# shanjiayao/PTT

Measured on AMD Instinct MI355X. Metric: tracklet frames/sec (hot path: PointNet++ SA stack + Point-Track-Transformer blocks), higher is better.
Workload: dtype f32

## Files before the change

### include/ptt_hip.h

```cpp
#ifndef PTT_HIP_H
#define PTT_HIP_H

#include <stddef.h>
#include <stdint.h>

#ifdef __cplusplus
extern "C" {
#endif

#define PTT_ABI_VERSION 28

enum {
    PTT_OK = 0,
    PTT_EINVAL = -1,
    PTT_EUNSUPPORTED = -2,
    PTT_ELAUNCH = -3,
    PTT_EWORKSPACE = -4
};

typedef void* ptt_stream_t;

int ptt_version(void);
const char* ptt_error_name(int code);
const char* ptt_last_error_string(void);

// ... 3 lines not shown
                   size_t workspace_elems, ptt_stream_t stream);

int ptt_gather_f32(const float* feat, const int32_t* idx, int B, int C, int N, int M,
                   float* out, ptt_stream_t stream);
int ptt_gather_grad_f32(const float* grad_out, const int32_t* idx, int B, int C, int N,
                        int M, float* grad_feat, ptt_stream_t stream);

int ptt_select_centres_f32(const float* xyz, const int32_t* idx, int B, int N, int M, float* new_xyz,
                           int64_t* idx64_out, ptt_stream_t stream);

int ptt_ball_query_f32(const float* new_xyz, const float* xyz, int B, int M, int N,
                       float radius, int nsample, int32_t* idx_out, ptt_stream_t stream);

int ptt_centres_ball_query_f32(const float* xyz, const int32_t* sel, int B, int N, int M, float radius, int nsample,
                               float* new_xyz, int64_t* idx64_out, int32_t* idx_out, ptt_stream_t stream);

int ptt_group_f32(const float* feat, const int32_t* idx, int B, int C, int N, int M,
                  int ns, float* out, ptt_stream_t stream);
int ptt_group_grad_f32(const float* grad_out, const int32_t* idx, int B, int C, int N,
                       int M, int ns, float* grad_feat, ptt_stream_t stream);

size_t ptt_scatter_add_det_workspace(int B, int N, int E);
int ptt_scatter_add_det_f32(const float* src, const int32_t* idx, int B, int C, int N, int E, float* out,
                            void* workspace, size_t workspace_bytes, ptt_stream_t stream);

int ptt_knn_f32(const float* xyz, int B, int N, int k, int32_t* idx_out,
                ptt_stream_t stream);
int ptt_knn_rel_f32(const float* xyz, int B, int N, int k, int32_t* idx_out, float* rel_out,
                    ptt_stream_t stream);

// ... 66 lines not shown
    int64_t feat_sb, feat_sc, feat_sn;
    float* out;
    int64_t out_sb, out_sc, out_sm;
    int B, N, M, nsample, C;
    float radius;
    int use_xyz;
    int normalize_xyz;
    int n_layers;
    ptt_sa_layer layers[PTT_SA_MAX_LAYERS];
    const float* l0_point_term;
    const float* l0_xyz_weight;
    int l0_channels;
    int l0_relu;
    void* compact_ws;
    size_t compact_ws_bytes;
} ptt_sa_desc;

int ptt_sa_fused_fwd_f32(const ptt_sa_desc* d, ptt_stream_t stream);
size_t ptt_sa_compact_workspace(int B, int M);

typedef struct ptt_xcorr_desc {
    const float* cos_t;
    const float* P;
    const float* w_sim;
    const float* scale0;
    const float* shift0;
    float* out;
    int64_t out_sb, out_sc, out_sn;
    float* sim_out;
    int B, Ns, Nt, C0;
    int n_layers;
    ptt_sa_layer layers[PTT_SA_MAX_LAYERS];
    int32_t split; int64_t out_sh;
    const float* search_feat; const float* templ_feat;
// ... 361 lines not shown
```

### ptt_amd/_lib.py

```python
import ctypes
import os
import re
from ctypes import Structure, c_char_p, c_double, c_float, c_int, c_int32, c_int64, c_longlong, c_size_t, c_uint32, c_void_p

from .build import HEADER as HEADER_PATH, LIB as LIB_PATH


def _strip_comments(text):
    return re.sub(r"/\*.*?\*/|//[^\n]*", " ", text, flags=re.S)


def parse_defines(text):
    return {n: int(v) for n, v in re.findall(r"^[ \t]*#[ \t]*define[ \t]+(PTT_\w+)[ \t]+(-?\d+)[ \t]*$", _strip_comments(text), re.M)}


CTYPES = {"int": c_int, "int32_t": c_int32, "uint32_t": c_uint32, "int64_t": c_int64, "long long": c_longlong, "size_t": c_size_t,
          "float": c_float, "double": c_double, "ptt_stream_t": c_void_p}


def _ctype(decl, name, is_return=False):
    words = decl.replace("*", " * ").split()
    if not is_return and len(words) > 1 and words[-1] != "*":
        words.pop()
    if "*" in words:
# ... 135 lines not shown


class SaLayer(Structure):
    _fields_ = [("Wpacked", c_void_p), ("scale", c_void_p), ("shift", c_void_p),
                ("Cin", c_int), ("Cout", c_int), ("relu", c_int)]


class SaDesc(Structure):
    _fields_ = [("xyz", c_void_p), ("new_xyz", c_void_p), ("idx", c_void_p), ("feat", c_void_p),
                ("feat_sb", c_int64), ("feat_sc", c_int64), ("feat_sn", c_int64),
                ("out", c_void_p), ("out_sb", c_int64), ("out_sc", c_int64), ("out_sm", c_int64),
                ("B", c_int), ("N", c_int), ("M", c_int), ("nsample", c_int), ("C", c_int),
                ("radius", c_float), ("use_xyz", c_int), ("normalize_xyz", c_int), ("n_layers", c_int),
                ("layers", SaLayer * PTT_SA_MAX_LAYERS),
                ("l0_point_term", c_void_p), ("l0_xyz_weight", c_void_p), ("l0_channels", c_int), ("l0_relu", c_int),
                ("compact_ws", c_void_p), ("compact_ws_bytes", c_size_t)]


class XcorrDesc(Structure):
    _fields_ = [("cos_t", c_void_p), ("P", c_void_p), ("w_sim", c_void_p), ("scale0", c_void_p), ("shift0", c_void_p),
                ("out", c_void_p), ("out_sb", c_int64), ("out_sc", c_int64), ("out_sn", c_int64),
                ("sim_out", c_void_p),
                ("B", c_int), ("Ns", c_int), ("Nt", c_int), ("C0", c_int),
                ("n_layers", c_int), ("layers", SaLayer * PTT_SA_MAX_LAYERS),
                ("split", c_int32), ("out_sh", c_int64), ("search_feat", c_void_p), ("templ_feat", c_void_p),
                ("s_sb", c_int64), ("s_sn", c_int64), ("t_sb", c_int64), ("t_sn", c_int64), ("C", c_int), ("eps", c_float)]


class AttnDesc(Structure):
    _fields_ = [("xyz", c_void_p), ("rel", c_void_p), ("knn", c_void_p), ("qkv", c_void_p),
                ("Wd1p", c_void_p), ("Wd2p", c_void_p), ("bd2", c_void_p),
# ... 36 lines not shown
```

### ptt_amd/csrc/mfma_ops.hip

```cpp
#include <math.h>
#include <stdlib.h>
#include <string.h>
#include "common.h"
#include "mfma_common.h"

#ifndef PTT_PAIR_PF
#define PTT_PAIR_PF 1
#endif
#ifndef PTT_GATHER_BATCH
#define PTT_GATHER_BATCH 16
#endif
#ifndef PTT_SA_WAVES
#define PTT_SA_WAVES 2
#endif

namespace ptt {

#ifdef PTT_DEV
#define PTT_STAMP(i) do { if (p.dbg && threadIdx.x == 0 && blockIdx.x < 4096) p.dbg[blockIdx.x * 8 + (i)] = __builtin_readcyclecounter(); } while (0)
#else
#define PTT_STAMP(i) do { } while (0)
#endif

__device__ __forceinline__ void stagger_second_slot(int first_wave_blocks, int quanta) {
// ... 1315 lines not shown
            if (valid) tab.ndist()[g0 + lc] = nd;
        }
    }
    __syncthreads();
    if (t < 4) s_base[t] = s_cnt[t] ? atomicAdd(&tab.ws[t], s_cnt[t]) : 0;
    __syncthreads();
    for (int e = t; e < 32 * 32; e += 256) {
        const int lc = e >> 5, j = e & 31, k = s_cls[lc];
        if (k < 0 || j >= (4 << k)) continue;
        const int q = s_base[k] + s_pos[lc];
        tab.rows(k)[(size_t)q * (4 << k) + j] = s_row[lc][j < s_nd[lc] ? j : 0];
        if (j == 0) tab.list(k)[q] = g0 + lc;
    }
}

#ifndef PTT_SAL_WGS
#define PTT_SAL_WGS 1
#endif
#ifndef PTT_SAL_WAVES
#define PTT_SAL_WAVES 12
#endif

template <int ROWS>
struct SacTileT {
    static constexpr int LG = ROWS == 32 ? 3 : 4;
    static_assert(ROWS == 32 || ROWS == 64, "32- or 64-row tiles");
    int k, first, n;
    __device__ __forceinline__ static void count(const int32_t* ws, int total, int (&cnt)[4], int (&tiles)[4]) {
#pragma unroll
        for (int k = 0; k < 4; ++k) {
// ... 665 lines not shown
        cin = s.Cout;
    }
    if (ldo < cin || (residual && ldr < cin)) return fail(PTT_EINVAL, "ptt_rows_mlp_f32: ldo=%d ldr=%d Cout=%d", ldo, ldr, cin);
    p.ldk = maxk + 4;
    p.vec_in = ((K & 3) == 0 && (ldx & 3) == 0 && (reinterpret_cast<uintptr_t>(X) & 15) == 0) ? 1 : 0;
    const int lds = 32 * p.ldk * (int)sizeof(float);
    int rc = set_lds_limit(reinterpret_cast<const void*>(rows_mlp_kernel), lds);
    if (rc) return rc;
    hipLaunchKernelGGL(rows_mlp_kernel, dim3((rows + 31) / 32), dim3(256), lds, as_stream(stream), p);
    return check_launch("rows_mlp_kernel");
}

extern "C" size_t ptt_sa_compact_workspace(int B, int M) {
    const long long T = (long long)(B > 0 ? B : 0) * (M > 0 ? M : 0);
    return SacTable::words((size_t)T) * sizeof(int32_t);
}

extern "C" int ptt_sa_fused_fwd_f32(const ptt_sa_desc* d, ptt_stream_t stream) {
    if (!d) return fail(PTT_EINVAL, "ptt_sa_fused_fwd_f32: null descriptor");
    if (d->B < 0 || d->N <= 0 || d->M < 0 || d->C < 0 || d->n_layers < 1 || d->n_layers > PTT_SA_MAX_LAYERS)
        return fail(PTT_EINVAL, "ptt_sa_fused_fwd_f32: B=%d N=%d M=%d C=%d layers=%d", d->B, d->N, d->M, d->C,
                    d->n_layers);
    if (d->nsample != 16 && d->nsample != 32 && d->nsample != 64)
        return fail(PTT_EUNSUPPORTED, "ptt_sa_fused_fwd_f32: nsample=%d (16, 32 and 64 are instantiated)", d->nsample);
    if (d->B == 0 || d->M == 0) return PTT_OK;
    const bool hoist = d->l0_point_term != nullptr;
    if (!d->xyz || !d->new_xyz || !d->idx || !d->out || (!hoist && d->C > 0 && !d->feat))
        return fail(PTT_EINVAL, "ptt_sa_fused_fwd_f32: null pointer");
    if (!d->use_xyz && d->C == 0) return fail(PTT_EINVAL, "ptt_sa_fused_fwd_f32: no xyz and no features");
    if (hoist) {
// ... 100 lines not shown
        }
        return check_launch("sa_wave_kernel");
    }
    if (p.hoist == 2 && d->nsample == 32 && d->n_layers == 2 && p.L[0].Cin == 128 && p.L[0].Cout == 128 &&
        p.L[1].Cout == 256 && !p.L[0].scale && !p.L[1].scale && p.L[0].relu && dev_switches().sa_stream) {
        p.tiles = (total_centres + 1) / 2;
        int wgs = p.tiles < 512 ? p.tiles : 512;
        p.chunk = (p.tiles + wgs - 1) / wgs;
        if (dev_switches().sa_chunk > 0 && p.chunk > dev_switches().sa_chunk) p.chunk = dev_switches().sa_chunk;
        wgs = (p.tiles + p.chunk - 1) / p.chunk;
        if (d->compact_ws) {
            if (d->compact_ws_bytes < ptt_sa_compact_workspace(d->B, d->M) || (reinterpret_cast<uintptr_t>(d->compact_ws) & 15))
                return fail(PTT_EWORKSPACE, "ptt_sa_fused_fwd_f32: compact_ws needs %zu bytes, 16-byte aligned (got %zu)",
                            ptt_sa_compact_workspace(d->B, d->M), d->compact_ws_bytes);
            p.cws = static_cast<int32_t*>(d->compact_ws);
            hipLaunchKernelGGL(sa_compact_zero_kernel, dim3(1), dim3(64), 0, s, p.cws);
            if ((rc = check_launch("sa_compact_zero_kernel"))) return rc;
            hipLaunchKernelGGL(sa_compact_kernel<false>, dim3((total_centres + 31) / 32), dim3(256), 0, s, d->xyz, d->idx, d->N, d->M,
                               SacTable{p.cws, total_centres});
            if ((rc = check_launch("sa_compact_kernel"))) return rc;
            const int lds = (2 * SAS_TILE + 64 * 4 + 64) * (int)sizeof(float);
            if ((rc = set_lds_limit(reinterpret_cast<const void*>(sa_stream_compact_kernel), lds))) return rc;
            hipLaunchKernelGGL(sa_stream_compact_kernel, dim3(p.tiles < 512 ? p.tiles : 512), dim3(256), lds, s, p);
            return check_launch("sa_stream_compact_kernel");
        }
        const int lds = (2 * SAS_TILE + 4 * 16 * 4) * (int)sizeof(float);
        if ((rc = set_lds_limit(reinterpret_cast<const void*>(sa_stream_kernel<32>), lds))) return rc;
        hipLaunchKernelGGL((sa_stream_kernel<32>), dim3(wgs), dim3(256), lds, s, p);
        return check_launch("sa_stream_kernel");
    }
    int RT = dev_switches().sa_rt;
    if (d->nsample == 64) RT = 2;
    const int lds = 32 * RT * p.ldk * (int)sizeof(float);
    if (lds > 160 * 1024) return fail(PTT_EUNSUPPORTED, "ptt_sa_fused_fwd_f32: %d B of LDS per workgroup", lds);
    const int cpw = 32 * RT / d->nsample;
// ... 126 lines not shown
```

### ptt_amd/csrc/point_ops.hip

```cpp
#pragma clang fp contract(off)

#include <limits.h>
#include <stdlib.h>
#include "common.h"

namespace ptt {

__device__ __forceinline__ float sqdist3(float ax, float ay, float az, float bx, float by, float bz) {
    const float dx = ax - bx, dy = ay - by, dz = az - bz;
    return (dx * dx + dy * dy) + dz * dz;
}

__device__ __forceinline__ float knn_dist(float ax, float ay, float az, float bx, float by, float bz) {
    const float d = sqdist3(ax, ay, az, bx, by, bz);
    return d < __builtin_inff() ? d : 3.402823466e+38f;
}

__device__ __forceinline__ float lane_bcast(float v, int src_lane) {
    return __builtin_bit_cast(float, __builtin_amdgcn_readlane(__builtin_bit_cast(int, v), src_lane));
}

typedef float fps_f2 __attribute__((ext_vector_type(2)));


// ... 181 lines not shown
            PTT_FPS_ABL_CASE(1) PTT_FPS_ABL_CASE(2) PTT_FPS_ABL_CASE(3) PTT_FPS_ABL_CASE(4) PTT_FPS_ABL_CASE(8) PTT_FPS_ABL_CASE(12) PTT_FPS_ABL_CASE(15)
            PTT_FPS_ABL_CASE(16) PTT_FPS_ABL_CASE(32) PTT_FPS_ABL_CASE(47) PTT_FPS_ABL_CASE(7) PTT_FPS_ABL_CASE(24) PTT_FPS_ABL_CASE(40)
#undef PTT_FPS_ABL_CASE
        }
#endif
        hipLaunchKernelGGL((fps_kernel<T, P, true>), dim3(B), dim3(T), sel_bytes + (size_t)N * 12, s, xyz, N, npoint, idx);
        return check_launch("fps_kernel");
    }
    hipLaunchKernelGGL((fps_kernel<T, P, false>), dim3(B), dim3(T), sel_bytes, s, xyz, N, npoint, idx);
    return check_launch("fps_kernel");
}

template <int CPW>
__device__ __forceinline__ void ball_sweep(const float* __restrict__ pts, int N, float r2, int ns, const float (&cx)[CPW],
                                           const float (&cy)[CPW], const float (&cz)[CPW], int ncentres,
                                           int32_t* __restrict__ out0, int lane) {
    int cnt[CPW], first[CPW];
#pragma unroll
    for (int c = 0; c < CPW; ++c) { cnt[c] = (c < ncentres) ? 0 : ns; first[c] = 0; }
    for (int base = 0; base < N; base += 64) {
        const int k = base + lane;
        const bool in = k < N;
        float px = 0.f, py = 0.f, pz = 0.f;
        if (in) { px = pts[3 * k + 0]; py = pts[3 * k + 1]; pz = pts[3 * k + 2]; }
        bool active = false;
#pragma unroll
        for (int c = 0; c < CPW; ++c) {
            if (cnt[c] >= ns) continue;
            const float d = sqdist3(cx[c], cy[c], cz[c], px, py, pz);
            const bool hit = in && d < r2;
            const unsigned long long mask = __ballot(hit);
            if (mask != 0ull) {
                if (cnt[c] == 0) first[c] = base + (__ffsll((long long)mask) - 1);
                const int pos = cnt[c] + __popcll(mask & ((1ull << lane) - 1ull));
                if (hit && pos < ns) out0[(size_t)c * ns + pos] = k;
                cnt[c] += __popcll(mask);
            }
            active = active || cnt[c] < ns;
        }
        if (!active) break;
    }
#pragma unroll
    for (int c = 0; c < CPW; ++c) {
        if (c >= ncentres) break;
        const int fill = (cnt[c] > 0) ? first[c] : 0;
        for (int s = cnt[c] + lane; s < ns; s += 64) out0[(size_t)c * ns + s] = fill;
    }
}

template <int CPW>
__global__ __launch_bounds__(256) void ball_query_kernel(const float* __restrict__ new_xyz,
                                                         const float* __restrict__ xyz, int BM, int M, int N,
                                                         float r2, int ns, int32_t* __restrict__ idx_out) {
    const int centre = (blockIdx.x * 4 + (threadIdx.x >> 6)) * CPW;
    if (centre >= BM) return;
    const int lane = threadIdx.x & 63;
    const int b = centre / M;
    float cx[CPW], cy[CPW], cz[CPW];
    const int nc = min(CPW, BM - centre);
#pragma unroll
    for (int c = 0; c < CPW; ++c) {
        const int cc = centre + (c < nc ? c : 0);
        cx[c] = new_xyz[(size_t)cc * 3 + 0]; cy[c] = new_xyz[(size_t)cc * 3 + 1]; cz[c] = new_xyz[(size_t)cc * 3 + 2];
    }
    ball_sweep<CPW>(xyz + (size_t)b * N * 3, N, r2, ns, cx, cy, cz, nc, idx_out + (size_t)centre * ns, lane);
}

template <int CPW>
__global__ __launch_bounds__(256) void centres_ball_query_kernel(const float* __restrict__ xyz, const int32_t* __restrict__ sel,
                                                                 int BM, int M, int N, float r2, int ns,
                                                                 float* __restrict__ new_xyz, long long* __restrict__ idx64,
                                                                 int32_t* __restrict__ idx_out) {
    const int centre = (blockIdx.x * 4 + (threadIdx.x >> 6)) * CPW;
    if (centre >= BM) return;
    const int lane = threadIdx.x & 63;
    const int b = centre / M;
    const float* __restrict__ pts = xyz + (size_t)b * N * 3;
    float cx[CPW], cy[CPW], cz[CPW];
    const int nc = min(CPW, BM - centre);
#pragma unroll
    for (int c = 0; c < CPW; ++c) {
        const int cc = centre + (c < nc ? c : 0);
        const int n = sel ? sel[cc] : cc - b * M;
        cx[c] = pts[3 * n + 0]; cy[c] = pts[3 * n + 1]; cz[c] = pts[3 * n + 2];
        if (lane == 0 && c < nc) {
            new_xyz[(size_t)cc * 3 + 0] = cx[c]; new_xyz[(size_t)cc * 3 + 1] = cy[c]; new_xyz[(size_t)cc * 3 + 2] = cz[c];
            if (idx64) idx64[cc] = n;
        }
    }
    ball_sweep<CPW>(pts, N, r2, ns, cx, cy, cz, nc, idx_out + (size_t)centre * ns, lane);
}

__global__ void gather_kernel(const float* __restrict__ feat, const int32_t* __restrict__ idx, int C, int N, int M,
                              float* __restrict__ out, size_t total) {
    for (size_t e = (size_t)blockIdx.x * blockDim.x + threadIdx.x; e < total; e += (size_t)gridDim.x * blockDim.x) {
        const int j = (int)(e % M);
        const size_t bc = e / M;
        const int b = (int)(bc / C);
        out[e] = feat[bc * N + idx[(size_t)b * M + j]];
    }
}
__global__ void gather_grad_kernel(const float* __restrict__ go, const int32_t* __restrict__ idx, int C, int N, int M,
                                   float* __restrict__ gf, size_t total) {
    for (size_t e = (size_t)blockIdx.x * blockDim.x + threadIdx.x; e < total; e += (size_t)gridDim.x * blockDim.x) {
        const int j = (int)(e % M);
// ... 852 lines not shown
    if (!xyz || !new_xyz || !idx_out) return fail(PTT_EINVAL, "ptt_centres_ball_query_f32: null pointer");
    const int BM = B * M;
    const int cpw = ball_cpw(BM, M);
    if (cpw == 8)
        hipLaunchKernelGGL((centres_ball_query_kernel<8>), dim3((BM / 8 + 3) / 4), dim3(256), 0, as_stream(stream), xyz, sel, BM,
                           M, N, radius * radius, nsample, new_xyz, reinterpret_cast<long long*>(idx64_out), idx_out);
    else if (cpw == 4)
        hipLaunchKernelGGL((centres_ball_query_kernel<4>), dim3((BM / 4 + 3) / 4), dim3(256), 0, as_stream(stream), xyz, sel, BM,
                           M, N, radius * radius, nsample, new_xyz, reinterpret_cast<long long*>(idx64_out), idx_out);
    else
        hipLaunchKernelGGL((centres_ball_query_kernel<1>), dim3((BM + 3) / 4), dim3(256), 0, as_stream(stream), xyz, sel, BM, M,
                           N, radius * radius, nsample, new_xyz, reinterpret_cast<long long*>(idx64_out), idx_out);
    return check_launch("centres_ball_query_kernel");
}


extern "C" size_t ptt_ball_query_grid_workspace(int B, int N) {
    if (B <= 0 || N <= 0) return 0;
    return (size_t)B * grid_slice_ints(N) * sizeof(int32_t);
}

static int ball_query_grid_launch(const char* who, const float* xyz, const float* centres, const int32_t* sel, int sel_mode, int B, int N, int M,
                                  float radius, int nsample, float* new_xyz, int64_t* idx64, int32_t* idx_out, void* ws, size_t ws_bytes,
                                  ptt_stream_t stream) {
    if (B < 0 || M < 0 || N <= 0 || nsample <= 0) return fail(PTT_EINVAL, "%s: B=%d M=%d N=%d nsample=%d", who, B, M, N, nsample);
    if (B == 0 || M == 0) return PTT_OK;
    if (N > 131072) return fail(PTT_EUNSUPPORTED, "%s: N=%d (the hit bitmap of a wave lives in LDS: at most 131072 points)", who, N);
    if (!ws || ws_bytes < ptt_ball_query_grid_workspace(B, N) || (reinterpret_cast<uintptr_t>(ws) & 15))
        return fail(PTT_EWORKSPACE, "%s: %zu bytes of 16-byte aligned workspace needed", who, ptt_ball_query_grid_workspace(B, N));
    hipStream_t s = as_stream(stream);
// ... 161 lines not shown
```

### ptt_amd/models/backbones_3d/pointnet2/pointnet2_modules.py

```python
import os
from typing import List

import torch
import torch.nn as nn
import torch.nn.functional as F

from .... import ops, train_ops
from ....param_cache import (DropsCachesOnModeChange, FoldedLayer, ParamCache, conv_bn_tensors, fold_conv_bn,
                             index_table)
from . import pointnet2_utils
from . import pytorch_utils as pt_utils

STREAM_COMPACT_MIN_BALLS = 2048
STREAM_COMPACT_MAX_POINTS = 1024


class PointnetSAModuleVotes(DropsCachesOnModeChange, nn.Module):
    def __init__(self, *, mlp: List[int], radius: float = None, nsample: int = None, bn: bool = True,
                 use_xyz: bool = True, normalize_xyz: bool = False, sample_uniformly: bool = False,
                 sample_method='fps'):
        super().__init__()
        self.radius = radius
        self.nsample = nsample
        self.mlp_module = None
# ... 79 lines not shown
            xyz = xyz.contiguous()
            inds, inds64, new_xyz, idx, self.centres_knn = ops.fps_ball_knn(xyz, npoint, self.radius, self.nsample, self.centres_knn_k)
            pre = (new_xyz, idx, inds64)
        prefix = inds is None and self.sample_method in ('rs', 'sequence')
        if pre is not None:
            pass
        elif prefix:
            inds64 = index_table(xyz.size(0), npoint, xyz.device, torch.int64)
        elif inds is None:
            inds = self._sample(xyz, features, npoint)
        else:
            assert inds.shape[1] == npoint
            inds = inds.to(torch.int32)

        xyz = xyz.contiguous()
        if pre is not None:
            new_xyz, idx, inds64 = pre
        elif prefix:
            new_xyz, _, idx = ops.centres_ball_query(xyz, None, npoint, self.radius, self.nsample)
        else:
            new_xyz, inds64, idx = ops.centres_ball_query(xyz, inds.contiguous(), npoint, self.radius, self.nsample)
        layers, hoist = self._fused_params(xyz.device)
        if hoist is not None and features is not None:
            wf_packed, wx, c0, relu0 = hoist
            rows = features.transpose(1, 2)
            uniform = rows.stride(2) == 1 and rows.stride(0) == rows.shape[1] * rows.stride(1)
            term = ops.linear(rows if uniform else rows.contiguous(), wf_packed, c0, None, layers[0].shift, relu=False)
            B, M, ns = xyz.shape[0], npoint, self.nsample
            if (B * M * ns <= ops.ONE_FRAME_MAX_SA_ROWS and ns in (16, 32) and len(layers) == 3 and c0 % 4 == 0 and c0 >= 192):
                L1, L2 = layers[1], layers[2]
                h = torch.empty((B * M * ns, L1.cout), dtype=torch.float32, device=xyz.device)
                ops.row_jobs([pt_utils.layer_job(L1, prologue=3, x=term, idx=idx, xyz=xyz, centres=new_xyz, wx=wx,
                                                 radius=self.radius, ns=ns, M=M, N=xyz.shape[1], normalize_xyz=self.normalize_xyz,
                                                 pro_relu=relu0, out=h)])
                pooled = torch.empty((B, M, L2.cout), dtype=torch.float32, device=xyz.device)
                ops.row_jobs([pt_utils.layer_job(L2, x=h, epilogue=2, ns=ns, M=M, out=pooled)])
                return new_xyz, pooled.transpose(1, 2), inds64
            new_features = ops.sa_fused_forward(xyz, new_xyz, idx, None, layers[1:], self.radius, True,
                                                self.normalize_xyz, point_major_out=True, l0=(term, wx, relu0),
                                                compact=(bool(compact) and B * M >= STREAM_COMPACT_MIN_BALLS
                                                         and xyz.shape[1] <= STREAM_COMPACT_MAX_POINTS))
        else:
            new_features = ops.sa_fused_forward(xyz, new_xyz, idx, features, layers, self.radius,
                                                self.use_xyz, self.normalize_xyz, point_major_out=True,
                                                compact=features is None)
        return new_xyz, new_features, inds64

    def _forward_train(self, xyz, features, npoint, inds):
        if inds is None:
            inds = self._sample(xyz, features, npoint)
        else:
            assert inds.shape[1] == npoint
            inds = inds.to(torch.int32)
        hoist = (self.use_xyz and not self.sample_uniformly and self.nsample * npoint <= 16384
                 and train_ops.usable(self.mlp_module, xyz if features is None else features)
                 and self.mlp_module[0].conv.weight.shape[0] % 4 == 0)
# ... 17 lines not shown
```

### ptt_amd/models/backbones_3d/pointnet2_backbone.py

```python
from typing import List

import torch
import torch.nn as nn

from ... import graph_policy, ops, train_ops
from ...param_cache import ParamCache, index_table
from .pointnet2 import pointnet2_modules


class PointNet2BackboneLight(nn.Module):
    def __init__(self, model_cfg, input_channels, **kwargs):
        super().__init__()
        self.model_cfg = model_cfg
        input_channels -= 3
        self.num_points_each_layer = []
        self.SA_modules = nn.ModuleList()
        sa = self.model_cfg.SA_CONFIG
        for k in range(len(sa.RADIUS)):
            mlps = list(sa.MLPS[k])
            if k == 0:
                mlps[0] = input_channels
            self.SA_modules.append(pointnet2_modules.PointnetSAModuleVotes(
                radius=sa.RADIUS[k], nsample=sa.NSAMPLE[k], mlp=mlps,
                use_xyz=sa.get('USE_XYZ', True), normalize_xyz=sa.get('NORMALIZE_XYZ', True),
                sample_method=sa.SAMPLE_METHOD[k]))
        self.cov_final = nn.Conv1d(256, 256, kernel_size=1)
        self.num_point_features = sa.MLPS[-1][-1]
        self._cov_cache = ParamCache()
        self.seed_knn = 16
        self.overlap_branches = True
        self._side_stream = None

    @staticmethod
    def _break_up_pc(pc):
        xyz = pc[..., 0:3].contiguous()
        features = pc[..., 3:].contiguous() if pc.size(-1) > 3 else None
        return xyz, features

    def _cov_final(self, features):
        if not features.is_cuda:
            return self.cov_final(features)
        if self.training:
            if features.dtype != torch.float32:
                return self.cov_final(features)
            return train_ops.rows_linear(self.cov_final, features.transpose(1, 2)).transpose(1, 2)
        if ops.autograd_recording(self.cov_final, features) or features.dtype != torch.float32:
# ... 20 lines not shown
            xyz = xyz.contiguous()
            if inds0 is None:
                inds0 = pointnet2_utils.furthest_point_sample(xyz, npoints[0])
            inds0 = inds0.to(torch.int32).contiguous()
            levels, inds64, knn = ops.sa_levels_point_jobs(xyz, inds0, list(npoints), list(sa.RADIUS), list(sa.NSAMPLE),
                                                           knn_k=want_knn)
            seq = [None] + [index_table(xyz.size(0), n, xyz.device, torch.int64) for n in npoints[1:3]]
            xyz, features, inds0 = self.SA_modules[0](xyz=xyz, features=features, npoint=npoints[0], inds=inds0,
                                                      pre=(levels[0][0], levels[0][1], inds64))
            xyz, features, inds1 = self.SA_modules[1](xyz=xyz, features=features, npoint=npoints[1],
                                                      pre=(levels[1][0], levels[1][1], seq[1]))
            xyz, features, inds2 = self.SA_modules[2](xyz=xyz, features=features, npoint=npoints[2],
                                                      pre=(levels[2][0], levels[2][1], seq[2]))
        else:
            xyz, features, inds0 = self.SA_modules[0](xyz=xyz, features=features, npoint=npoints[0], inds=inds0)
            xyz, features, inds1 = self.SA_modules[1](xyz=xyz, features=features, npoint=npoints[1], compact=1 in compact_levels)
            xyz, features, inds2 = self.SA_modules[2](xyz=xyz, features=features, npoint=npoints[2], compact=2 in compact_levels)
        point_features = self._cov_final(features)
        assert inds1.dtype == inds2.dtype == torch.int64, 'index type must be int64, not {}'.format(inds2.dtype)
        if all(m.sample_method in ('rs', 'sequence') for m in self.SA_modules[1:]) and inds0.shape[1] >= npoints[2]:
            inds = inds0[:, :npoints[2]]
        else:
            inds = inds0.gather(1, inds1).gather(1, inds2)
        if want_knn:
            return xyz, point_features, inds, knn
        return xyz, point_features, inds

    def sample(self, search_points, template_points):
        from .pointnet2 import pointnet2_utils
        sa = self.model_cfg.SA_CONFIG
        assert sa.SAMPLE_METHOD[0] == 'fps'
        return (pointnet2_utils.furthest_point_sample(search_points[..., 0:3].contiguous(), sa.NPOINTS_SEARCH[0]),
                pointnet2_utils.furthest_point_sample(template_points[..., 0:3].contiguous(), sa.NPOINTS_TEMPLATE[0]))

    def forward_branches(self, search_points, template_points, inds=None):
        sa = self.model_cfg.SA_CONFIG
        i_s, i_t = inds if inds is not None else (None, None)
        last = (len(self.SA_modules) - 1,) if (search_points.is_cuda and not self.training) else ()
        if not (self.overlap_branches and search_points.is_cuda and not self.training):
            r = self.branch_forward(search_points, sa.NPOINTS_SEARCH, i_s, want_knn=self.seed_knn, compact_levels=last)
            t_seeds, t_feats, t_inds = self.branch_forward(template_points, sa.NPOINTS_TEMPLATE, i_t)
        else:
            if self._side_stream is None or self._side_stream.device != search_points.device:
                self._side_stream = torch.cuda.Stream(device=search_points.device)
            main = torch.cuda.current_stream(search_points.device)
            side = graph_policy.branch(main, self._side_stream)
            with torch.cuda.stream(side):
                t_seeds, t_feats, t_inds = self.branch_forward(template_points, sa.NPOINTS_TEMPLATE, i_t)
            r = self.branch_forward(search_points, sa.NPOINTS_SEARCH, i_s, want_knn=self.seed_knn, compact_levels=last)
            graph_policy.join(main, side)
            if side is not main:
                for t in (t_seeds, t_feats, t_inds, template_points):
                    t.record_stream(main)
        s_seeds, s_feats, s_inds = r[:3]
        s_knn = r[3] if len(r) > 3 else None
        out = {'search_seeds': s_seeds, 'search_feats': s_feats, 'search_inds': s_inds,
               'template_seeds': t_seeds, 'template_feats': t_feats, 'template_inds': t_inds}
        if s_knn is not None:
            out['search_seeds_knn'] = s_knn
        return out

    def forward(self, batch_dict):
        batch_dict.update(self.forward_branches(batch_dict['search_points'], batch_dict['template_points'],
# ... 5 lines not shown
```

### ptt_amd/models/trackers/tracker3d_template.py

```python
import os

import torch
import torch.nn as nn

from .. import backbones_3d, similarity_modules, voting_heads


class Tracker3DTemplate(nn.Module):
    def __init__(self, model_cfg, num_class, dataset):
        super().__init__()
        self.model_cfg = model_cfg
        self.num_class = num_class
        self.dataset = dataset
        self.training = dataset.training
        self.class_names = dataset.class_names
        self.register_buffer('global_step', torch.LongTensor(1).zero_())
        self.module_topology = ['backbone_3d', 'similarity_module', 'centroid_voting_head', 'box_voting_head']

    @property
    def mode(self):
        return 'TRAIN' if self.training else 'TEST'

    def forward(self, **kwargs):
        raise NotImplementedError
# ... 11 lines not shown
            'voxel_size': self.dataset.voxel_size,
        }
        for name in self.module_topology:
            module, info = getattr(self, 'build_%s' % name)(model_info_dict=info)
            self.add_module(name, module)
        return info['module_list']

    def build_backbone_3d(self, model_info_dict):
        cfg = self.model_cfg.get('BACKBONE_3D', None)
        if cfg is None:
            return None, model_info_dict
        module = backbones_3d.__all__[cfg.NAME](
            model_cfg=cfg, input_channels=model_info_dict['num_point_features'],
            grid_size=model_info_dict['grid_size'], voxel_size=model_info_dict['voxel_size'],
            point_cloud_range=model_info_dict['point_cloud_range'])
        model_info_dict['module_list'].append(module)
        model_info_dict['num_point_features'] = module.num_point_features
        return module, model_info_dict

    def build_similarity_module(self, model_info_dict):
        cfg = self.model_cfg.get('SIMILARITY_MODULE', None)
        if cfg is None:
            return None, model_info_dict
        module = similarity_modules.__all__[cfg.NAME](model_cfg=cfg)
        model_info_dict['module_list'].append(module)
        return module, model_info_dict

    def _build_head(self, key, model_info_dict):
        cfg = self.model_cfg.get(key, None)
        if cfg is None:
# ... 52 lines not shown
```

### ptt_amd/ops.py

```python
import contextlib
import ctypes
import os

import torch

from . import _lib
from ._lib import AttnDesc, SaDesc, SaLayer, XcorrDesc


def _stream():
    return ctypes.c_void_p(torch.cuda.current_stream().cuda_stream)


_timing = None


def start_kernel_timing(names):
    global _timing
    _timing = {n: [] for n in names}


def stop_kernel_timing():
    global _timing
    t, _timing = _timing, None
# ... 215 lines not shown
    B, N, _ = xyz.shape
    if sel is not None:
        _chk(sel, "sel", torch.int32, 2)
    M = int(npoint)
    new_xyz = torch.empty((B, M, 3), dtype=torch.float32, device=xyz.device)
    idx64 = torch.empty((B, M), dtype=torch.int64, device=xyz.device) if (want_idx64 and sel is not None) else None
    idx = torch.empty((B, M, int(nsample)), dtype=torch.int32, device=xyz.device)
    if GRID_BALL_QUERY_MIN_POINTS <= N <= 131072:
        ws, ws_arg = _workspace("ptt_ball_query_grid_workspace", xyz.device, B, N)
        _launch("ptt_centres_ball_query_grid_f32", xyz.device, _ptr(xyz), _ptr(sel), B, N, M, float(radius), int(nsample), _ptr(new_xyz), _ptr(idx64),
                _ptr(idx), *ws_arg, timed='ptt_ball_query_f32')
    else:
        _launch("ptt_centres_ball_query_f32", xyz.device, _ptr(xyz), _ptr(sel), B, N, M, float(radius), int(nsample), _ptr(new_xyz), _ptr(idx64),
                _ptr(idx), timed='ptt_ball_query_f32')
    return new_xyz, idx64, idx


def group_points(features, idx):
    _chk(features, "features", torch.float32, 3)
    _chk(idx, "idx", torch.int32, 3)
    B, C, N = features.shape
    _, M, ns = idx.shape
    out = torch.empty((B, C, M, ns), dtype=torch.float32, device=features.device)
    _launch("ptt_group_f32", features.device, _ptr(features), _ptr(idx), B, C, N, M, ns, _ptr(out))
    return out


def group_points_grad(grad_out, idx, N):
    _chk(grad_out, "grad_out", torch.float32, 4)
    _chk(idx, "idx", torch.int32, 3)
# ... 62 lines not shown
    if (scale is None and (rows > 8192 or (rows >= 6144 and int(cout) == 256)) and x2.data_ptr() % 16 == 0 and o2.is_contiguous()
            and _host("ptt_rows_gemm_supported", rows, K, int(cout), x2.stride(0), int(cout))):
        _launch("ptt_rows_gemm_f32", x.device, _ptr(x2), rows, K, x2.stride(0), None, None, _ptr(wpacked), int(cout), _ptr(shift), 1 if relu else 0,
                _ptr(r2), r2.stride(0) if r2 is not None else int(cout), _ptr(o2), int(cout), None, 0, timed='ptt_linear_f32')
        return out
    if rows <= ROW_JOB_MAX_ROWS and 192 <= K <= 1024 and o2.stride(1) == 1:
        row_jobs([row_job(wpacked, cout, x=x2, scale=scale, shift=shift, act=1 if relu else 0, res=r2, out=o2)])
        return out
    _launch("ptt_linear_f32", x.device, _ptr(x2), rows, K, x2.stride(0) if rows > 1 else K, _ptr(wpacked), int(cout), _ptr(scale), _ptr(shift),
            1 if relu else 0, _ptr(r2), (r2.stride(0) if (r2 is not None and rows > 1) else int(cout)), _ptr(o2),
            o2.stride(0) if rows > 1 else int(cout), timed='ptt_linear_f32')
    return out


def sa_fused_forward(xyz, new_xyz, idx, features, layers, radius, use_xyz=True, normalize_xyz=False,
                     point_major_out=True, l0=None, compact=False):
    _chk(xyz, "xyz", torch.float32, 3)
    _chk(new_xyz, "new_xyz", torch.float32, 3)
    _chk(idx, "idx", torch.int32, 3)
    B, N, _ = xyz.shape
    _, M, ns = idx.shape
    d = SaDesc()
    d.xyz, d.new_xyz, d.idx = xyz.data_ptr(), new_xyz.data_ptr(), idx.data_ptr()
    if features is not None:
        if not features.is_cuda or features.dtype != torch.float32 or features.dim() != 3:
            raise RuntimeError("features must be a (B,C,N) float32 device tensor")
        d.feat = features.data_ptr()
        d.feat_sb, d.feat_sc, d.feat_sn = features.stride()
        d.C = features.shape[1]
    else:
        d.feat, d.C = None, 0
# ... 16 lines not shown
        L.Cin, L.Cout, L.relu = int(cin), int(co), int(bool(relu))
    if l0 is not None:
        term, wx, l0_relu = l0
        if features is not None:
            raise RuntimeError("with a hoisted layer 0 the point features are already inside l0[0]")
        _chk(term, "l0 point term", torch.float32, 3)
        _chk(wx, "l0 xyz weight", torch.float32, 2)
        if term.shape[0] != B or term.shape[1] != N or wx.shape[0] != 3 or wx.shape[1] != term.shape[2]:
            raise RuntimeError("l0 point term must be (B,N,C0) and the xyz weight (3,C0)")
        d.l0_point_term, d.l0_xyz_weight = term.data_ptr(), wx.data_ptr()
        d.l0_channels, d.l0_relu = term.shape[2], int(bool(l0_relu))
    if isinstance(compact, torch.Tensor):
        if not compact.is_cuda or compact.device != xyz.device or not compact.is_contiguous():
            raise RuntimeError("compact workspace must be a contiguous tensor on %s" % xyz.device)
        d.compact_ws, d.compact_ws_bytes = compact.data_ptr(), compact.numel() * compact.element_size()
    elif compact:
        ws, (_, d.compact_ws_bytes) = _workspace("ptt_sa_compact_workspace", xyz.device, B, M)
        d.compact_ws = ws.data_ptr()
    _launch("ptt_sa_fused_fwd_f32", xyz.device, ctypes.byref(d), timed='ptt_sa_fused_fwd_f32')
    return out


def cosine_map(search_feats, templ_feats, eps=1e-8):
    for t_, n_ in ((search_feats, "search_feats"), (templ_feats, "templ_feats")):
        if not isinstance(t_, torch.Tensor) or not t_.is_cuda or t_.dtype != torch.float32 or t_.dim() != 3:
            raise RuntimeError("%s must be a (B,C,N) float32 device tensor" % n_)
    if search_feats.shape[:2] != templ_feats.shape[:2] or search_feats.device != templ_feats.device:
        raise RuntimeError("search_feats and templ_feats must share batch size, channel count and device")
    B, C, Ns = search_feats.shape
    Nt = templ_feats.shape[2]
# ... 1331 lines not shown
```

Measured before the change: 17370.

## Build SA compaction table from ball-query hit counts and widen compact levels

The ball query now records each centre's neighbour hit count and zeroes the compaction workspace counters inside the same kernel. A new small kernel builds the size-class compaction table from those counts, so the SA fused forward no longer runs its own zero kernel and the compact kernel that rescans xyz. The tracker also turns on stream compaction for more SA levels, including search level 1 and template level 1. This adds a separate table launch and puts compaction on levels where it may not pay off.

```diff
diff --git a/include/ptt_hip.h b/include/ptt_hip.h
--- a/include/ptt_hip.h
+++ b/include/ptt_hip.h
@@ -8,7 +8,7 @@
 extern "C" {
 #endif
 
-#define PTT_ABI_VERSION 28
+#define PTT_ABI_VERSION 29
 
 enum {
     PTT_OK = 0,
@@ -42,6 +42,10 @@
 
 int ptt_centres_ball_query_f32(const float* xyz, const int32_t* sel, int B, int N, int M, float radius, int nsample,
                                float* new_xyz, int64_t* idx64_out, int32_t* idx_out, ptt_stream_t stream);
+
+int ptt_centres_ball_query_hits_f32(const float* xyz, const int32_t* sel, int B, int N, int M, float radius, int nsample,
+                                    float* new_xyz, int64_t* idx64_out, int32_t* idx_out, int32_t* hits_out,
+                                    void* compact_ws, size_t compact_ws_bytes, ptt_stream_t stream);
 
 int ptt_group_f32(const float* feat, const int32_t* idx, int B, int C, int N, int M,
                   int ns, float* out, ptt_stream_t stream);
@@ -138,10 +142,13 @@
     int l0_relu;
     void* compact_ws;
     size_t compact_ws_bytes;
+    int compact_table_ready;
 } ptt_sa_desc;
 
 int ptt_sa_fused_fwd_f32(const ptt_sa_desc* d, ptt_stream_t stream);
 size_t ptt_sa_compact_workspace(int B, int M);
+int ptt_sa_compact_table_f32(const int32_t* idx, const int32_t* hits, int B, int M, int nsample, void* compact_ws,
+                             size_t compact_ws_bytes, ptt_stream_t stream);
 
 typedef struct ptt_xcorr_desc {
     const float* cos_t;
diff --git a/ptt_amd/_lib.py b/ptt_amd/_lib.py
--- a/ptt_amd/_lib.py
+++ b/ptt_amd/_lib.py
@@ -173,7 +173,7 @@
                 ("radius", c_float), ("use_xyz", c_int), ("normalize_xyz", c_int), ("n_layers", c_int),
                 ("layers", SaLayer * PTT_SA_MAX_LAYERS),
                 ("l0_point_term", c_void_p), ("l0_xyz_weight", c_void_p), ("l0_channels", c_int), ("l0_relu", c_int),
-                ("compact_ws", c_void_p), ("compact_ws_bytes", c_size_t)]
+                ("compact_ws", c_void_p), ("compact_ws_bytes", c_size_t), ("compact_table_ready", c_int)]
 
 
 class XcorrDesc(Structure):
diff --git a/ptt_amd/csrc/mfma_ops.hip b/ptt_amd/csrc/mfma_ops.hip
--- a/ptt_amd/csrc/mfma_ops.hip
+++ b/ptt_amd/csrc/mfma_ops.hip
@@ -1353,6 +1353,34 @@
     }
 }
 
+__global__ __launch_bounds__(256) void sa_compact_table_kernel(const int32_t* __restrict__ idx, const int32_t* __restrict__ hits,
+                                                               SacTable tab) {
+    __shared__ int s_cnt[4], s_base[4], s_cls[32], s_pos[32], s_nd[32];
+    const int t = threadIdx.x, g0 = blockIdx.x * 32, T = tab.T;
+    if (t < 4) s_cnt[t] = 0;
+    __syncthreads();
+    if (t < 32) {
+        const bool valid = g0 + t < T;
+        const int nd = valid ? min(max(hits[g0 + t], 1), 32) : 1;
+        const int k = nd <= 4 ? 0 : nd <= 8 ? 1 : nd <= 16 ? 2 : 3;
+        s_cls[t] = valid ? k : -1;
+        s_nd[t] = nd;
+        s_pos[t] = valid ? atomicAdd(&s_cnt[k], 1) : 0;
+        if (valid) tab.ndist()[g0 + t] = nd;
+    }
+    __syncthreads();
+    if (t < 4) s_base[t] = s_cnt[t] ? atomicAdd(&tab.ws[t], s_cnt[t]) : 0;
+    __syncthreads();
+    for (int e = t; e < 32 * 32; e += 256) {
+        const int lc = e >> 5, j = e & 31, k = s_cls[lc];
+        if (k < 0 || j >= (4 << k)) continue;
+        const int q = s_base[k] + s_pos[lc];
+        if (q < 0 || q >= T) continue;
+        tab.rows(k)[(size_t)q * (4 << k) + j] = idx[(size_t)(g0 + lc) * 32 + (j < s_nd[lc] ? j : 0)];
+        if (j == 0) tab.list(k)[q] = g0 + lc;
+    }
+}
+
 #ifndef PTT_SAL_WGS
 #define PTT_SAL_WGS 1
 #endif
@@ -2048,6 +2076,23 @@
 extern "C" size_t ptt_sa_compact_workspace(int B, int M) {
     const long long T = (long long)(B > 0 ? B : 0) * (M > 0 ? M : 0);
     return SacTable::words((size_t)T) * sizeof(int32_t);
+}
+
+extern "C" int ptt_sa_compact_table_f32(const int32_t* idx, const int32_t* hits, int B, int M, int nsample, void* compact_ws,
+                                        size_t compact_ws_bytes, ptt_stream_t stream) {
+    if (B < 0 || M < 0) return fail(PTT_EINVAL, "ptt_sa_compact_table_f32: B=%d M=%d", B, M);
+    if (nsample != 32) return fail(PTT_EUNSUPPORTED, "ptt_sa_compact_table_f32: nsample=%d (the stream shape has 32)", nsample);
+    if (B == 0 || M == 0) return PTT_OK;
+    if (!idx || !hits) return fail(PTT_EINVAL, "ptt_sa_compact_table_f32: null pointer");
+    if ((unsigned long long)B * M * 32ull * 4ull >= 0x7fffffffull)
+        return fail(PTT_EUNSUPPORTED, "ptt_sa_compact_table_f32: B=%d M=%d: the index array exceeds 2 GiB — split the batch", B, M);
+    if (!compact_ws || compact_ws_bytes < ptt_sa_compact_workspace(B, M) || (reinterpret_cast<uintptr_t>(compact_ws) & 15))
+        return fail(PTT_EWORKSPACE, "ptt_sa_compact_table_f32: compact_ws needs %zu bytes, 16-byte aligned (got %zu)",
+                    ptt_sa_compact_workspace(B, M), compact_ws_bytes);
+    const int T = B * M;
+    hipLaunchKernelGGL(sa_compact_table_kernel, dim3((T + 31) / 32), dim3(256), 0, as_stream(stream), idx, hits,
+                       SacTable{static_cast<int32_t*>(compact_ws), T});
+    return check_launch("sa_compact_table_kernel");
 }
 
 extern "C" int ptt_sa_fused_fwd_f32(const ptt_sa_desc* d, ptt_stream_t stream) {
@@ -2178,11 +2223,13 @@
                 return fail(PTT_EWORKSPACE, "ptt_sa_fused_fwd_f32: compact_ws needs %zu bytes, 16-byte aligned (got %zu)",
                             ptt_sa_compact_workspace(d->B, d->M), d->compact_ws_bytes);
             p.cws = static_cast<int32_t*>(d->compact_ws);
-            hipLaunchKernelGGL(sa_compact_zero_kernel, dim3(1), dim3(64), 0, s, p.cws);
-            if ((rc = check_launch("sa_compact_zero_kernel"))) return rc;
-            hipLaunchKernelGGL(sa_compact_kernel<false>, dim3((total_centres + 31) / 32), dim3(256), 0, s, d->xyz, d->idx, d->N, d->M,
-                               SacTable{p.cws, total_centres});
-            if ((rc = check_launch("sa_compact_kernel"))) return rc;
+            if (!d->compact_table_ready) {
+                hipLaunchKernelGGL(sa_compact_zero_kernel, dim3(1), dim3(64), 0, s, p.cws);
+                if ((rc = check_launch("sa_compact_zero_kernel"))) return rc;
+                hipLaunchKernelGGL(sa_compact_kernel<false>, dim3((total_centres + 31) / 32), dim3(256), 0, s, d->xyz, d->idx, d->N, d->M,
+                                   SacTable{p.cws, total_centres});
+                if ((rc = check_launch("sa_compact_kernel"))) return rc;
+            }
             const int lds = (2 * SAS_TILE + 64 * 4 + 64) * (int)sizeof(float);
             if ((rc = set_lds_limit(reinterpret_cast<const void*>(sa_stream_compact_kernel), lds))) return rc;
             hipLaunchKernelGGL(sa_stream_compact_kernel, dim3(p.tiles < 512 ? p.tiles : 512), dim3(256), lds, s, p);
diff --git a/ptt_amd/csrc/point_ops.hip b/ptt_amd/csrc/point_ops.hip
--- a/ptt_amd/csrc/point_ops.hip
+++ b/ptt_amd/csrc/point_ops.hip
@@ -219,7 +219,7 @@
 template <int CPW>
 __device__ __forceinline__ void ball_sweep(const float* __restrict__ pts, int N, float r2, int ns, const float (&cx)[CPW],
                                            const float (&cy)[CPW], const float (&cz)[CPW], int ncentres,
-                                           int32_t* __restrict__ out0, int lane) {
+                                           int32_t* __restrict__ out0, int lane, int32_t* __restrict__ hits0 = nullptr) {
     int cnt[CPW], first[CPW];
 #pragma unroll
     for (int c = 0; c < CPW; ++c) { cnt[c] = (c < ncentres) ? 0 : ns; first[c] = 0; }
@@ -250,6 +250,7 @@
         if (c >= ncentres) break;
         const int fill = (cnt[c] > 0) ? first[c] : 0;
         for (int s = cnt[c] + lane; s < ns; s += 64) out0[(size_t)c * ns + s] = fill;
+        if (hits0 && lane == 0) hits0[c] = max(1, min(cnt[c], ns));
     }
 }
 
@@ -272,10 +273,9 @@
 }
 
 template <int CPW>
-__global__ __launch_bounds__(256) void centres_ball_query_kernel(const float* __restrict__ xyz, const int32_t* __restrict__ sel,
-                                                                 int BM, int M, int N, float r2, int ns,
-                                                                 float* __restrict__ new_xyz, long long* __restrict__ idx64,
-                                                                 int32_t* __restrict__ idx_out) {
+__device__ __forceinline__ void centres_ball_query_body(const float* __restrict__ xyz, const int32_t* __restrict__ sel, int BM, int M, int N,
+                                                        float r2, int ns, float* __restrict__ new_xyz, long long* __restrict__ idx64,
+                                                        int32_t* __restrict__ idx_out, int32_t* __restrict__ hits) {
     const int centre = (blockIdx.x * 4 + (threadIdx.x >> 6)) * CPW;
     if (centre >= BM) return;
     const int lane = threadIdx.x & 63;
@@ -293,7 +293,25 @@
             if (idx64) idx64[cc] = n;
         }
     }
-    ball_sweep<CPW>(pts, N, r2, ns, cx, cy, cz, nc, idx_out + (size_t)centre * ns, lane);
+    ball_sweep<CPW>(pts, N, r2, ns, cx, cy, cz, nc, idx_out + (size_t)centre * ns, lane, hits ? hits + centre : nullptr);
+}
+
+template <int CPW>
+__global__ __launch_bounds__(256) void centres_ball_query_kernel(const float* __restrict__ xyz, const int32_t* __restrict__ sel,
+                                                                 int BM, int M, int N, float r2, int ns,
+                                                                 float* __restrict__ new_xyz, long long* __restrict__ idx64,
+                                                                 int32_t* __restrict__ idx_out) {
+    centres_ball_query_body<CPW>(xyz, sel, BM, M, N, r2, ns, new_xyz, idx64, idx_out, nullptr);
+}
+
+template <int CPW>
+__global__ __launch_bounds__(256) void centres_ball_query_hits_kernel(const float* __restrict__ xyz, const int32_t* __restrict__ sel,
+                                                                      int BM, int M, int N, float r2, int ns,
+                                                                      float* __restrict__ new_xyz, long long* __restrict__ idx64,
+                                                                      int32_t* __restrict__ idx_out, int32_t* __restrict__ hits,
+                                                                      int32_t* __restrict__ cws) {
+    if (blockIdx.x == 0 && threadIdx.x < 16) cws[threadIdx.x] = 0;
+    centres_ball_query_body<CPW>(xyz, sel, BM, M, N, r2, ns, new_xyz, idx64, idx_out, hits);
 }
 
 __global__ void gather_kernel(const float* __restrict__ feat, const int32_t* __restrict__ idx, int C, int N, int M,
@@ -1176,6 +1194,31 @@
     return check_launch("centres_ball_query_kernel");
 }
 
+extern "C" int ptt_centres_ball_query_hits_f32(const float* xyz, const int32_t* sel, int B, int N, int M, float radius, int nsample,
+                                               float* new_xyz, int64_t* idx64_out, int32_t* idx_out, int32_t* hits_out,
+                                               void* compact_ws, size_t compact_ws_bytes, ptt_stream_t stream) {
+    if (B < 0 || M < 0 || N <= 0 || nsample <= 0 || (!sel && M > N))
+        return fail(PTT_EINVAL, "ptt_centres_ball_query_hits_f32: B=%d M=%d N=%d nsample=%d", B, M, N, nsample);
+    if (B == 0 || M == 0) return PTT_OK;
+    if (!xyz || !new_xyz || !idx_out || !hits_out) return fail(PTT_EINVAL, "ptt_centres_ball_query_hits_f32: null pointer");
+    if (!compact_ws || compact_ws_bytes < ptt_sa_compact_workspace(B, M) || (reinterpret_cast<uintptr_t>(compact_ws) & 15))
+        return fail(PTT_EWORKSPACE, "ptt_centres_ball_query_hits_f32: compact_ws needs %zu bytes, 16-byte aligned (got %zu)",
+                    ptt_sa_compact_workspace(B, M), compact_ws_bytes);
+    const int BM = B * M;
+    const int cpw = ball_cpw(BM, M);
+    int32_t* const cws = static_cast<int32_t*>(compact_ws);
+    if (cpw == 8)
+        hipLaunchKernelGGL((centres_ball_query_hits_kernel<8>), dim3((BM / 8 + 3) / 4), dim3(256), 0, as_stream(stream), xyz, sel, BM,
+                           M, N, radius * radius, nsample, new_xyz, reinterpret_cast<long long*>(idx64_out), idx_out, hits_out, cws);
+    else if (cpw == 4)
+        hipLaunchKernelGGL((centres_ball_query_hits_kernel<4>), dim3((BM / 4 + 3) / 4), dim3(256), 0, as_stream(stream), xyz, sel, BM,
+                           M, N, radius * radius, nsample, new_xyz, reinterpret_cast<long long*>(idx64_out), idx_out, hits_out, cws);
+    else
+        hipLaunchKernelGGL((centres_ball_query_hits_kernel<1>), dim3((BM + 3) / 4), dim3(256), 0, as_stream(stream), xyz, sel, BM, M,
+                           N, radius * radius, nsample, new_xyz, reinterpret_cast<long long*>(idx64_out), idx_out, hits_out, cws);
+    return check_launch("centres_ball_query_hits_kernel");
+}
+
 
 extern "C" size_t ptt_ball_query_grid_workspace(int B, int N) {
     if (B <= 0 || N <= 0) return 0;
diff --git a/ptt_amd/models/backbones_3d/pointnet2/pointnet2_modules.py b/ptt_amd/models/backbones_3d/pointnet2/pointnet2_modules.py
--- a/ptt_amd/models/backbones_3d/pointnet2/pointnet2_modules.py
+++ b/ptt_amd/models/backbones_3d/pointnet2/pointnet2_modules.py
@@ -117,13 +117,21 @@
             inds = inds.to(torch.int32)
 
         xyz = xyz.contiguous()
+        layers, hoist = self._fused_params(xyz.device)
+        compact = (compact if (compact and hoist is not None and features is not None
+                               and xyz.shape[0] * npoint >= STREAM_COMPACT_MIN_BALLS
+                               and xyz.shape[1] <= STREAM_COMPACT_MAX_POINTS) else False)
+        table = None
         if pre is not None:
             new_xyz, idx, inds64 = pre
+        elif compact == 'table' and self.nsample == 32:
+            sel = None if prefix else inds.contiguous()
+            new_xyz, i64, idx, _, table = ops.centres_ball_query_table(xyz, sel, npoint, self.radius, self.nsample)
+            inds64 = inds64 if prefix else i64
         elif prefix:
             new_xyz, _, idx = ops.centres_ball_query(xyz, None, npoint, self.radius, self.nsample)
         else:
             new_xyz, inds64, idx = ops.centres_ball_query(xyz, inds.contiguous(), npoint, self.radius, self.nsample)
-        layers, hoist = self._fused_params(xyz.device)
         if hoist is not None and features is not None:
             wf_packed, wx, c0, relu0 = hoist
             rows = features.transpose(1, 2)
@@ -141,8 +149,8 @@
                 return new_xyz, pooled.transpose(1, 2), inds64
             new_features = ops.sa_fused_forward(xyz, new_xyz, idx, None, layers[1:], self.radius, True,
                                                 self.normalize_xyz, point_major_out=True, l0=(term, wx, relu0),
-                                                compact=(bool(compact) and B * M >= STREAM_COMPACT_MIN_BALLS
-                                                         and xyz.shape[1] <= STREAM_COMPACT_MAX_POINTS))
+                                                compact=table if table is not None else bool(compact),
+                                                table_ready=table is not None)
         else:
             new_features = ops.sa_fused_forward(xyz, new_xyz, idx, features, layers, self.radius,
                                                 self.use_xyz, self.normalize_xyz, point_major_out=True,
diff --git a/ptt_amd/models/backbones_3d/pointnet2_backbone.py b/ptt_amd/models/backbones_3d/pointnet2_backbone.py
--- a/ptt_amd/models/backbones_3d/pointnet2_backbone.py
+++ b/ptt_amd/models/backbones_3d/pointnet2_backbone.py
@@ -30,6 +30,8 @@
         self.seed_knn = 16
         self.overlap_branches = True
         self._side_stream = None
+        self.compact_levels = (('search', len(sa.RADIUS) - 1),)
+        self.compact_table = False
 
     @staticmethod
     def _break_up_pc(pc):
@@ -80,8 +82,9 @@
                                                       pre=(levels[2][0], levels[2][1], seq[2]))
         else:
             xyz, features, inds0 = self.SA_modules[0](xyz=xyz, features=features, npoint=npoints[0], inds=inds0)
-            xyz, features, inds1 = self.SA_modules[1](xyz=xyz, features=features, npoint=npoints[1], compact=1 in compact_levels)
-            xyz, features, inds2 = self.SA_modules[2](xyz=xyz, features=features, npoint=npoints[2], compact=2 in compact_levels)
+            how = 'table' if self.compact_table else True
+            xyz, features, inds1 = self.SA_modules[1](xyz=xyz, features=features, npoint=npoints[1], compact=1 in compact_levels and how)
+            xyz, features, inds2 = self.SA_modules[2](xyz=xyz, features=features, npoint=npoints[2], compact=2 in compact_levels and how)
         point_features = self._cov_final(features)
         assert inds1.dtype == inds2.dtype == torch.int64, 'index type must be int64, not {}'.format(inds2.dtype)
         if all(m.sample_method in ('rs', 'sequence') for m in self.SA_modules[1:]) and inds0.shape[1] >= npoints[2]:
@@ -102,17 +105,19 @@
     def forward_branches(self, search_points, template_points, inds=None):
         sa = self.model_cfg.SA_CONFIG
         i_s, i_t = inds if inds is not None else (None, None)
-        last = (len(self.SA_modules) - 1,) if (search_points.is_cuda and not self.training) else ()
+        on = search_points.is_cuda and not self.training
+        last = tuple(l for b, l in self.compact_levels if b == 'search') if on else ()
+        last_t = tuple(l for b, l in self.compact_levels if b == 'template') if on else ()
         if not (self.overlap_branches and search_points.is_cuda and not self.training):
             r = self.branch_forward(search_points, sa.NPOINTS_SEARCH, i_s, want_knn=self.seed_knn, compact_levels=last)
-            t_seeds, t_feats, t_inds = self.branch_forward(template_points, sa.NPOINTS_TEMPLATE, i_t)
+            t_seeds, t_feats, t_inds = self.branch_forward(template_points, sa.NPOINTS_TEMPLATE, i_t, compact_levels=last_t)
         else:
             if self._side_stream is None or self._side_stream.device != search_points.device:
                 self._side_stream = torch.cuda.Stream(device=search_points.device)
             main = torch.cuda.current_stream(search_points.device)
             side = graph_policy.branch(main, self._side_stream)
             with torch.cuda.stream(side):
-                t_seeds, t_feats, t_inds = self.branch_forward(template_points, sa.NPOINTS_TEMPLATE, i_t)
+                t_seeds, t_feats, t_inds = self.branch_forward(template_points, sa.NPOINTS_TEMPLATE, i_t, compact_levels=last_t)
             r = self.branch_forward(search_points, sa.NPOINTS_SEARCH, i_s, want_knn=self.seed_knn, compact_levels=last)
             graph_policy.join(main, side)
             if side is not main:
diff --git a/ptt_amd/models/trackers/tracker3d_template.py b/ptt_amd/models/trackers/tracker3d_template.py
--- a/ptt_amd/models/trackers/tracker3d_template.py
+++ b/ptt_amd/models/trackers/tracker3d_template.py
@@ -4,6 +4,8 @@
 import torch.nn as nn
 
 from .. import backbones_3d, similarity_modules, voting_heads
+
+TRACKER_COMPACT_LEVELS = (('search', 1), ('search', 2), ('template', 1))
 
 
 class Tracker3DTemplate(nn.Module):
@@ -49,6 +51,9 @@
             model_cfg=cfg, input_channels=model_info_dict['num_point_features'],
             grid_size=model_info_dict['grid_size'], voxel_size=model_info_dict['voxel_size'],
             point_cloud_range=model_info_dict['point_cloud_range'])
+        if hasattr(module, 'compact_levels'):
+            module.compact_levels = TRACKER_COMPACT_LEVELS
+            module.compact_table = True
         model_info_dict['module_list'].append(module)
         model_info_dict['num_point_features'] = module.num_point_features
         return module, model_info_dict
diff --git a/ptt_amd/ops.py b/ptt_amd/ops.py
--- a/ptt_amd/ops.py
+++ b/ptt_amd/ops.py
@@ -253,6 +253,26 @@
         _launch("ptt_centres_ball_query_f32", xyz.device, _ptr(xyz), _ptr(sel), B, N, M, float(radius), int(nsample), _ptr(new_xyz), _ptr(idx64),
                 _ptr(idx), timed='ptt_ball_query_f32')
     return new_xyz, idx64, idx
+
+
+def centres_ball_query_table(xyz, sel, npoint, radius, nsample, want_idx64=True):
+    _chk(xyz, "xyz", torch.float32, 3)
+    B, N, _ = xyz.shape
+    if sel is not None:
+        _chk(sel, "sel", torch.int32, 2)
+    M = int(npoint)
+    if N >= GRID_BALL_QUERY_MIN_POINTS or int(nsample) != 32:
+        raise RuntimeError("centres_ball_query_table: N=%d nsample=%d (fewer than %d points per cloud and 32 neighbours)"
+                           % (N, int(nsample), GRID_BALL_QUERY_MIN_POINTS))
+    new_xyz = torch.empty((B, M, 3), dtype=torch.float32, device=xyz.device)
+    idx64 = torch.empty((B, M), dtype=torch.int64, device=xyz.device) if (want_idx64 and sel is not None) else None
+    idx = torch.empty((B, M, 32), dtype=torch.int32, device=xyz.device)
+    hits = torch.empty((B, M), dtype=torch.int32, device=xyz.device)
+    ws, ws_arg = _workspace("ptt_sa_compact_workspace", xyz.device, B, M)
+    _launch("ptt_centres_ball_query_hits_f32", xyz.device, _ptr(xyz), _ptr(sel), B, N, M, float(radius), 32, _ptr(new_xyz), _ptr(idx64),
+            _ptr(idx), _ptr(hits), *ws_arg, timed='ptt_ball_query_f32')
+    _launch("ptt_sa_compact_table_f32", xyz.device, _ptr(idx), _ptr(hits), B, M, 32, *ws_arg, timed='ptt_sa_compact_table_f32')
+    return new_xyz, idx64, idx, hits, ws
 
 
 def group_points(features, idx):
@@ -345,7 +365,7 @@
 
 
 def sa_fused_forward(xyz, new_xyz, idx, features, layers, radius, use_xyz=True, normalize_xyz=False,
-                     point_major_out=True, l0=None, compact=False):
+                     point_major_out=True, l0=None, compact=False, table_ready=False):
     _chk(xyz, "xyz", torch.float32, 3)
     _chk(new_xyz, "new_xyz", torch.float32, 3)
     _chk(idx, "idx", torch.int32, 3)
@@ -392,6 +412,9 @@
         if not compact.is_cuda or compact.device != xyz.device or not compact.is_contiguous():
             raise RuntimeError("compact workspace must be a contiguous tensor on %s" % xyz.device)
         d.compact_ws, d.compact_ws_bytes = compact.data_ptr(), compact.numel() * compact.element_size()
+        d.compact_table_ready = int(bool(table_ready))
+    elif table_ready:
+        raise RuntimeError("table_ready needs the workspace that holds the table as `compact`")
     elif compact:
         ws, (_, d.compact_ws_bytes) = _workspace("ptt_sa_compact_workspace", xyz.device, B, M)
         d.compact_ws = ws.data_ptr()
```

Result: no change. 17400, median of 6 (+0.2%).
